# jingsenzhu/i2-sdf

Measured on AMD Instinct MI355X. Metric: ray-samples/sec (fwd+bwd), higher is better.
Workload: dtype f32 (bf16x3 split MFMA: fp32 operands as 3 bf16 terms, fp32 accumulate; the 256x256 weight-gradient GEMM blocks and the sampler's depth-choosing sdf-only passes: 2 bf16 terms per operand, 3 products, fp32 accumulate; the saved SDF tensors abar / G(hbar) / G(a) -- operands of those GEMMs and of the s

## Files before the change

i2sdf_amd/csrc/pack.hip:

```cpp
#include "plan.h"

using namespace i2sdf;

int i2sdf_hip_check(hipError_t e, const char* what);

namespace {

struct RowTab {
  int32_t n;
  int32_t rows[3 * I2SDF_MAX_LAYERS], cols[3 * I2SDF_MAX_LAYERS], scale_off[3 * I2SDF_MAX_LAYERS];
  int64_t off_v[3 * I2SDF_MAX_LAYERS], off_g[3 * I2SDF_MAX_LAYERS];
};

__global__ __launch_bounds__(256) void rowscale_kernel(RowTab tab, const float* __restrict__ params, float* __restrict__ scale,
                                                        int n_rows) {
  const int row = blockIdx.x * 4 + (threadIdx.x >> 6);
  const int lane = threadIdx.x & 63;
  if (row >= n_rows) return;
  int e = 0;
  while (e + 1 < tab.n && row >= tab.scale_off[e + 1]) ++e;
  const int r = row - tab.scale_off[e];
  const int cols = tab.cols[e];
  const float* v = params + tab.off_v[e] + (int64_t)r * cols;
  float s = 0.f;
  for (int c = lane; c < cols; c += 64) { float x = v[c]; s = fmaf(x, x, s); }
#pragma unroll
  for (int o = 32; o > 0; o >>= 1) s += __shfl_xor(s, o);
  if (lane == 0) scale[row] = params[tab.off_g[e] + r] / sqrtf(s);
}

__device__ __forceinline__ int map_col(const ColMap& cm, int kp) {
  if (kp < cm.split) return kp < cm.valid0 ? cm.base0 + kp : -1;
  const int j = kp - cm.split;
  return j < cm.valid1 ? cm.base1 + j : -1;
}

__global__ __launch_bounds__(256) void pack_kernel(const Seg* __restrict__ segs, int n_segs, const float* __restrict__ params,
                                                    const float* __restrict__ scale, float* __restrict__ chunks,
                                                    int64_t total_chunks) {
  const int64_t gid = (int64_t)blockIdx.x * 256 + threadIdx.x;
  const int64_t chunk = gid >> 6;
  const int lane = (int)(gid & 63);
  if (chunk >= total_chunks) return;
  int lo = 0, hi_ = n_segs - 1;
  while (lo < hi_) {
    const int mid = (lo + hi_ + 1) >> 1;
    if (segs[mid].chunk0 <= chunk) lo = mid; else hi_ = mid - 1;
  }
  const Seg s = segs[lo];
  const int c = (int)(chunk - s.chunk0);
  const int i32 = lane & 31, hi = lane >> 5;
  f32x4 out = {0.f, 0.f, 0.f, 0.f};
  if (c < s.used) {
    if (s.type == SEG_BIAS) {
      const int nt = c / 4, q = c % 4;
#pragma unroll
      for (int t = 0; t < 4; ++t) {
        const int r = 32 * nt + 8 * q + 4 * hi + t;
        out[t] = (r < s.nrows) ? params[s.off_bias + s.row_off + r] : 0.f;
      }
    } else if (s.type == SEG_WFWD) {
      const int nt = c / s.KC, kc = c % s.KC;
      const int r = 32 * nt + i32;
      if (r < s.nrows) {
        const int row = s.row_off + r;
        const float sc = scale[s.scale_off + row] * s.mult;
        const float* v = params + s.off_v + (int64_t)row * s.cols;
#pragma unroll
        for (int t = 0; t < 4; ++t) {
          const int col = map_col(s.cm, 8 * kc + 4 * hi + t);
          out[t] = col >= 0 ? v[col] * sc : 0.f;
        }
      }
    } else if (s.type == SEG_WFWD3) {
      const int G = s.NT / 2, w = c >> 1, e = c & 1;
      const int kc = w / (3 * G), g = (w / 3) % G, sp = w % 3;
      const int r = 32 * (2 * g + e) + i32;
      unsigned q[4] = {0u, 0u, 0u, 0u};
      if (r < s.nrows) {
        const int row = s.row_off + r;
        const float sc = scale[s.scale_off + row] * s.mult;
        const float* v = params + s.off_v + (int64_t)row * s.cols;
#pragma unroll
        for (int i = 0; i < 4; ++i) {
          float x[2];
#pragma unroll
          for (int h2 = 0; h2 < 2; ++h2) {
            const int j = 2 * i + h2;
            const int col = map_col(s.cm, 16 * kc + (j & 3) + 8 * (j >> 2) + 4 * hi);
            x[h2] = col >= 0 ? v[col] * sc : 0.f;
          }
          unsigned p0, p1, p2;
          split3_pair(x[0], x[1], p0, p1, p2);
          q[i] = sp == 0 ? p0 : (sp == 1 ? p1 : p2);
        }
      }
// ... 37 lines not shown
      const int arow = 16 * (2 * g + e) + i16;
      const bool fwd = s.type != SEG_WBWD3H;
      const int acol = fwd ? -1 : map_col(s.cm, arow);
      unsigned q[4] = {0u, 0u, 0u, 0u};
      if (fwd ? (arow < s.nrows) : (acol >= 0)) {
#pragma unroll
        for (int i = 0; i < 4; ++i) {
          float x[2];
#pragma unroll
          for (int h2 = 0; h2 < 2; ++h2) {
            const int j = 2 * i + h2;
            const int k = 32 * kc + 16 * (j >> 2) + 4 * kg + (j & 3);
            x[h2] = 0.f;
            if (fwd) {
              const int row = s.row_off + arow, col = map_col(s.cm, k);
              if (col >= 0) x[h2] = params[s.off_v + (int64_t)row * s.cols + col] * (scale[s.scale_off + row] * s.mult);
            } else if (k < s.nrows) {
              const int row = s.row_off + k;
              x[h2] = params[s.off_v + (int64_t)row * s.cols + acol] * scale[s.scale_off + row] * s.mult;
            }
          }
          unsigned p0, p1, p2;
          split3_pair(x[0], x[1], p0, p1, p2);
          q[i] = sp == 0 ? p0 : (sp == 1 ? p1 : p2);
        }
      }
      out = __builtin_bit_cast(f32x4, u32x4{q[0], q[1], q[2], q[3]});
    } else if (s.type == SEG_ROWVEC_H) {
      const int rr = c / s.KC, nt = c % s.KC, kg = lane >> 4;
      const int row = s.row_off + rr;
      const float sc = scale[s.scale_off + row] * s.mult;
#pragma unroll
      for (int t = 0; t < 4; ++t) {
        const int col = map_col(s.cm, 16 * nt + 4 * kg + t);
        out[t] = col >= 0 ? params[s.off_v + (int64_t)row * s.cols + col] * sc : 0.f;
      }
    } else if (s.type == SEG_WBWD) {
      const int kt = c / s.KC, nc = c % s.KC;
      const int col = map_col(s.cm, 32 * kt + i32);
      if (col >= 0) {
#pragma unroll
        for (int t = 0; t < 4; ++t) {
          const int r = 8 * nc + 4 * hi + t;
          if (r < s.nrows) {
            const int row = s.row_off + r;
            out[t] = params[s.off_v + (int64_t)row * s.cols + col] * scale[s.scale_off + row] * s.mult;
          }
        }
      }
    } else if (s.type == SEG_ROWVEC) {
      const int rr = c / s.KC, kc = c % s.KC;
      const int row = s.row_off + rr;
      const float sc = scale[s.scale_off + row] * s.mult;
#pragma unroll
      for (int t = 0; t < 4; ++t) {
        const int col = map_col(s.cm, 8 * kc + 4 * hi + t);
        out[t] = col >= 0 ? params[s.off_v + (int64_t)row * s.cols + col] * sc : 0.f;
      }
    } else if (s.type == SEG_SCALAR) {
#pragma unroll
      for (int t = 0; t < 4; ++t) out[t] = (t < s.nrows) ? params[s.off_bias + s.row_off + t] : 0.f;
    }
  }
  reinterpret_cast<f32x4*>(chunks)[chunk * 64 + lane] = out;
}

void fill_tab(RowTab& tab, const NetPlan& np) {
  for (int l = 0; l < np.d.n_lin; ++l) {
    const int e = tab.n++;
    tab.rows[e] = np.d.out_dim[l]; tab.cols[e] = np.d.in_dim[l]; tab.scale_off[e] = np.scale_off[l];
    tab.off_v[e] = np.d.off_v[l]; tab.off_g[e] = np.d.off_g[l];
  }
}

}

extern "C" int i2sdf_pack_weights(const i2sdf_plan* p, const float* params, float* packed, void* stream) {
  if (!p || !params || !packed) return I2SDF_EINVAL;
  if (!p->d_segs) return I2SDF_EHIP;
  hipStream_t st = (hipStream_t)stream;
  RowTab tab{};
  fill_tab(tab, p->sdf); fill_tab(tab, p->rgb);
  if (p->light.d.n_lin) fill_tab(tab, p->light);
  rowscale_kernel<<<cdiv(p->n_scale, 4), 256, 0, st>>>(tab, params, packed, p->n_scale);
  const int64_t threads = p->total_chunks * 64;
  pack_kernel<<<(unsigned)((threads + 255) / 256), 256, 0, st>>>(p->d_segs, p->n_segs, params, packed, packed + p->scale_floats,
                                                                 p->total_chunks);
  return i2sdf_hip_check(hipGetLastError(), "pack_weights launch");
}
```

i2sdf_amd/csrc/plan.cpp:

```cpp
#include <hip/hip_runtime.h>
#include <string.h>
#include <initializer_list>
#include <string>
#include "plan.h"
#include <stdlib.h>

using namespace i2sdf;

static thread_local std::string g_hip_err;

int i2sdf_hip_check(hipError_t e, const char* what) {
  if (e == hipSuccess) return I2SDF_OK;
  g_hip_err = std::string(what) + ": " + hipGetErrorString(e);
  return I2SDF_EHIP;
}

extern "C" int i2sdf_version(void) { return I2SDF_VERSION; }
extern "C" const char* i2sdf_last_hip_error(void) { return g_hip_err.c_str(); }
extern "C" const char* i2sdf_strerror(int code) {
  switch (code) {
    case I2SDF_OK: return "ok";
    case I2SDF_EINVAL: return "invalid argument or unsupported network shape";
    case I2SDF_EHIP: return "HIP runtime error";
    case I2SDF_ESPHERE: return "ray misses the scene bounding sphere";
// ... 479 lines not shown
  }
  if (option == I2SDF_OPT_WGRAD_BF16X2) {
    p->wgrad_bf16x2 = value ? 1 : 0;
    return I2SDF_OK;
  }
  if (option == I2SDF_OPT_BLOCKED_SAVES) {
    p->blocked_saves = value ? 1 : 0;
    return I2SDF_OK;
  }
  if (option == I2SDF_OPT_SAVES24) {
    if (value && (p->H != 256 || p->F != 256 || span_chunks(p->sdf, SPAN_REV3_CHAIN) == 0)) return I2SDF_EINVAL;
    if (p->chain_active) return I2SDF_EINVAL;
    p->saves24 = value ? 1 : 0;
    return I2SDF_OK;
  }
  if (option == I2SDF_OPT_TAIL_OVERLAP) {
    p->tail_overlap = value ? 1 : 0;
    return I2SDF_OK;
  }
  return I2SDF_EINVAL;
}

extern "C" int i2sdf_plan_set_exchange(i2sdf_plan* p, const i2sdf_exchange* ex, int32_t flags) {
  if (!p || (flags & ~I2SDF_DP_GLOBAL_SAMPLER) || (ex && !ex->allreduce)) return I2SDF_EINVAL;
  p->exchange = ex ? *ex : i2sdf_exchange{nullptr, nullptr};
  p->dp_flags = ex ? flags : 0;
  return I2SDF_OK;
}

extern "C" int64_t i2sdf_plan_pack_floats(const i2sdf_plan* p) {
// ... 4 lines not shown
```

i2sdf_amd/csrc/plan.h:

```cpp
#pragma once
#include <stdint.h>
#include <vector>
#include "../../include/i2sdf.h"
#include "x3h.h"

namespace i2sdf {

enum SegType : int32_t { SEG_ZERO = 0, SEG_BIAS = 1, SEG_WFWD = 2, SEG_WBWD = 3, SEG_ROWVEC = 4, SEG_SCALAR = 5,
                         SEG_WFWD3 = 6 ,
                         SEG_WBWD3 = 7 ,
                         SEG_BIAS_H = 8, SEG_WFWD3H = 9, SEG_WBWD3H = 10, SEG_ROWVEC_H = 11,
                         SEG_WFWD2H = 12  };

struct ColMap { int32_t split, base0, valid0, base1, valid1; };

struct Seg {
  int64_t chunk0;
  int32_t nchunks;
  int32_t type;
  int64_t off_v, off_bias;
  int32_t scale_off;
  int32_t rows, cols;
  int32_t row_off;
  int32_t nrows;
// ... 51 lines not shown
  int64_t wgrad_floats = 0;
  int32_t H = 0, F = 0;
  int32_t n_cu = 256;
  int32_t rgb_bf16x3 = 0;
  int32_t sdf_bwd_bf16x3 = 0;
  int32_t train_fwd_bf16x3 = 0;
  int32_t wgrad_bf16x3 = 0;
  int32_t sdf_fwd_bf16x3 = 0;
  int32_t sampler_bf16x2 = 0;
  i2sdf_exchange exchange{nullptr, nullptr};
  int32_t dp_flags = 0;
  int32_t wgrad_bf16x2 = 0;
  int32_t blocked_saves = 0;
  int32_t saves24 = 0;
  int32_t tail_overlap = 0;
  mutable hipStream_t side = nullptr;
  mutable hipEvent_t ev_fork = nullptr, ev_join = nullptr;
  int32_t parts = 0;
  mutable hipStream_t part_st[I2SDF_MAX_PARTS - 1] = {nullptr, nullptr, nullptr};
  mutable hipEvent_t part_ev[I2SDF_MAX_PARTS] = {nullptr, nullptr, nullptr, nullptr};
  mutable int32_t chain_active = 0;
  mutable int64_t chain_M = 0;
};

namespace i2sdf {
struct Span { const float* w = nullptr; int n_stages = 0; };
inline int64_t span_chunks(const NetPlan& np, SpanId id) { return np.mark[id.to] - np.mark[id.from]; }
inline Span span(const i2sdf_plan* p, const float* packed, const NetPlan& np, SpanId id) {
  const int64_t n = span_chunks(np, id);
  if (n <= 0 || n % id.stage_chunks) return Span{};
// ... 63 lines not shown
```

i2sdf_amd/csrc/sampler.hip:

```cpp
#include "plan.h"

using namespace i2sdf;

int i2sdf_hip_check(hipError_t e, const char* what);

namespace {

constexpr int NMAX = 640;
constexpr int NNEW = 128;
constexpr int EMAX = NMAX / 64;

enum { ST_DONE = 0, ST_ITERS = 1, ST_FLAG0 = 2 , ST_CNT0 = 16 , ST_WORDS = 32 };

#ifndef SAMPLER_DPP
#define SAMPLER_DPP 1
#endif
template <int CTRL, int ROW_MASK>
__device__ __forceinline__ float dpp_mov(float old, float v) {
  return __builtin_bit_cast(float, __builtin_amdgcn_update_dpp(__builtin_bit_cast(int, old), __builtin_bit_cast(int, v), CTRL, ROW_MASK, 0xf, false));
}
constexpr int DPP_ROW_SHR1 = 0x111, DPP_ROW_SHR2 = 0x112, DPP_ROW_SHR4 = 0x114, DPP_ROW_SHR8 = 0x118, DPP_ROW_BCAST15 = 0x142, DPP_ROW_BCAST31 = 0x143;
__device__ __forceinline__ float wscan_incl(float v, int lane) {
#if SAMPLER_DPP
  (void)lane;
// ... 410 lines not shown
          const float x = buf[wv][i], y = buf[wv][l];
          const bool up = (i & k) == 0;
          if ((x > y) == up) { buf[wv][i] = y; buf[wv][l] = x; }
        }
      }
      __syncthreads();
    }
  }
  if (active) {
    for (int k = lane; k < total; k += 64) z_out[ray * ldz + k] = buf[wv][k];
    if (lane == 0 && z_eik) {
      int id = eik_idx ? eik_idx[ray] : 0;
      id = id < 0 ? 0 : (id > total - 1 ? total - 1 : id);
      z_eik[ray] = buf[wv][id];
    }
  }
}

template <int E>
__global__ __launch_bounds__(256) void error_bound_kernel(int64_t B, int n, const float* __restrict__ z, const float* __restrict__ sdf,
                                                           const float* __restrict__ beta, int64_t ldbeta, const float* __restrict__ d_star_in,
                                                           float* __restrict__ d_star_out, float* __restrict__ bound) {
  const int lane = threadIdx.x & 63;
  const int64_t ray = (int64_t)blockIdx.x * 4 + (threadIdx.x >> 6);
  if (ray >= B) return;
  Row<E> r;
  load_row<E>(r, z + ray * n, sdf + ray * n, n, lane);
  row_intervals<E>(r, lane);
#pragma unroll
  for (int e = 0; e < E; ++e) {
// ... 107 lines not shown
    int xrc = I2SDF_OK;
    switch (E) {
      case 1: xrc = launch_iter<1>(a, st, gcomm); break;
      case 2: xrc = launch_iter<2>(a, st, gcomm); break;
      case 3: xrc = launch_iter<3>(a, st, gcomm); break;
      case 4: xrc = launch_iter<4>(a, st, gcomm); break;
      case 5: xrc = launch_iter<5>(a, st, gcomm); break;
      case 6: xrc = launch_iter<6>(a, st, gcomm); break;
      case 7: xrc = launch_iter<7>(a, st, gcomm); break;
      case 8: xrc = launch_iter<8>(a, st, gcomm); break;
      case 9: xrc = launch_iter<9>(a, st, gcomm); break;
      default: xrc = launch_iter<10>(a, st, gcomm); break;
    }
    if (xrc) return xrc;
  }
  sampler_final_kernel<<<grid, 256, 0, st>>>(B, state, sc->N_samples_eval, zA, zB, samples, sc->N_samples, sc->N_samples_extra,
                                             training ? (const int*)extra_idx : nullptr, (const int*)extra_tab, near, far, (const int*)eik_idx, z_out, ldz,
                                             z_eik, iters_out);
  return i2sdf_hip_check(hipGetLastError(), "sample_rays launch");
}
```

i2sdf_amd/engine.py:

```python
from __future__ import annotations

import ctypes as C
from typing import Optional

import os

import torch

from . import lib as L
from .config import NetConfig
from .params import ParamLayout


class RenderEngine:
    def __init__(self, cfg: NetConfig, device="cuda"):
        self.cfg = cfg
        self.layout = ParamLayout(cfg)
        self.device = torch.device(device)
        self._lib = L.load()
        self._desc = self.layout.net_desc()
        plan = C.c_void_p()
        L.check(self._lib.i2sdf_plan_create(C.byref(self._desc), C.byref(plan)), "i2sdf_plan_create")
        self._plan = plan
        self.pack_floats = int(self._lib.i2sdf_plan_pack_floats(plan))
        self.wgrad_floats = int(self._lib.i2sdf_plan_wgrad_floats(plan))
        self.packed = torch.zeros(self.pack_floats, dtype=torch.float32, device=self.device)
        self._pack_stream, self._pack_event, self._pack_readers = None, None, {}
        self.F = cfg.feature_size
        wide = cfg.sdf.hidden == 256 and cfg.feature_size == 256
        self.set_sdf_forward_bf16x3(bool(cfg.bf16x3 and cfg.sdf.hidden % 64 == 0))
        self.set_wgrad_bf16x3(bool(cfg.bf16x3))
        self.set_train_forward_bf16x3(bool(cfg.bf16x3 and wide))
        self.set_sdf_backward_bf16x3(bool(cfg.bf16x3 and wide))
        self.set_rgb_bf16x3(bool(cfg.bf16x3 and cfg.rgb.hidden == 256 and cfg.feature_size == 256 and cfg.rgb.n_lin >= 3))
        self.wgrad_bf16x2 = False
        x2 = os.environ.get("I2SDF_WGRAD_BF16X2", "")
        self.set_wgrad_bf16x2(bool(cfg.bf16x3 and ((x2 != "0") if x2 != "" else cfg.wgrad_bf16x2)))
        self.sampler_bf16x2 = False
        sx2 = os.environ.get("I2SDF_SAMPLER_BF16X2", "")
        if wide:
            self.set_sampler_bf16x2(bool(self.sdf_forward_bf16x3 and ((sx2 != "0") if sx2 != "" else getattr(cfg, "sampler_bf16x2", False))))
        self.set_blocked_saves(bool(cfg.bf16x3 and os.environ.get("I2SDF_BLOCKED_SAVES", "1") != "0"))
        self.saves24 = False
        s24 = os.environ.get("I2SDF_SAVES24", "")
        if wide:
            self.set_saves24(bool(cfg.bf16x3 and ((s24 != "0") if s24 != "" else getattr(cfg, "saves24", True))))
        self.set_tail_overlap(os.environ.get("I2SDF_TAIL_OVERLAP", "1") != "0")
        self.parts = 0
        n_parts = int(os.environ.get("I2SDF_PARTS", "2"))
        self._parts_wanted = n_parts if (cfg.bf16x3 and n_parts >= 2) else 0
        self._sync_parts()
        sc = cfg.sampler
        self._scfg = L.SamplerCfg(near=sc.near, eps=sc.eps, add_tiny=sc.add_tiny, N_samples=sc.N_samples, N_samples_eval=sc.N_samples_eval,
                                  N_samples_extra=sc.N_samples_extra, beta_iters=sc.beta_iters, max_total_iters=sc.max_total_iters)
        dev = self.device
        self.t_lin = torch.linspace(0.0, 1.0, steps=sc.N_samples_eval, device=dev)
        self.u_more = torch.linspace(0.0, 1.0, steps=sc.N_samples_eval, device=dev)
        self.u_final = torch.linspace(0.0, 1.0, steps=sc.N_samples, device=dev)
        if sc.N_samples_extra > 0:
            self.extra_tab = torch.stack([torch.linspace(0, sc.N_samples_eval * (it + 1) - 1, sc.N_samples_extra).long()
                                          for it in range(sc.max_total_iters)]).to(torch.int32).to(dev).contiguous()
# ... 9 lines not shown
            def __init__(self, fn, name):
                self.fn, self.name = fn, name

            def __call__(self, *a):
                e0, e1 = torch.cuda.Event(enable_timing=True), torch.cuda.Event(enable_timing=True)
                e0.record()
                rc = self.fn(*a)
                e1.record()
                eng._timing.append((self.name, e0, e1))
                return rc

        self._timed_lib = type("TimedLib", (), {})()
        for name in L.SIGNATURES:
            fn = getattr(self._lib, name)
            if name in ("i2sdf_sdf_forward", "i2sdf_sdf_forward_grad", "i2sdf_rgb_forward", "i2sdf_rgb_backward", "i2sdf_sdf_backward",
                        "i2sdf_weight_grads", "i2sdf_sample_rays", "i2sdf_composite_forward", "i2sdf_composite_backward", "i2sdf_pack_weights",
                        "i2sdf_ray_setup", "i2sdf_light_forward", "i2sdf_light_backward"):
                fn = _Timed(fn, name)
            setattr(self._timed_lib, name, fn)
        self._real_lib, self._lib = self._lib, self._timed_lib

    def stop_timing(self):
        self._lib = self._real_lib
        out = {}
        for name, e0, e1 in self._timing:
            tot, cnt = out.get(name, (0.0, 0))
            out[name] = (tot + e0.elapsed_time(e1), cnt + 1)
        self._timing = []
        return out

    def __del__(self):
# ... 7 lines not shown
    def pack(self, flat_params: torch.Tensor):
        assert flat_params.is_cuda and flat_params.dtype == torch.float32 and flat_params.numel() == self.layout.n_params
        if os.environ.get("I2SDF_PACK_ASYNC", "1") == "0":
            L.check(self._lib.i2sdf_pack_weights(self._plan, L.ptr(flat_params), L.ptr(self.packed), L.stream_ptr()), "i2sdf_pack_weights")
            return
        dev = flat_params.device
        side = self._pack_stream
        if side is None:
            side = self._pack_stream = torch.cuda.Stream(device=dev)
        cur = torch.cuda.current_stream(dev)
        side.wait_stream(cur)
        for st in getattr(self, "_pack_readers", {}):
            if st != cur:
                side.wait_stream(st)
        with torch.cuda.stream(side):
            L.check(self._lib.i2sdf_pack_weights(self._plan, L.ptr(flat_params), L.ptr(self.packed), L.stream_ptr()), "i2sdf_pack_weights")
            self._pack_event = side.record_event()
        flat_params.record_stream(side)
        self._pack_readers = {}

    def _pk(self):
        ev = self._pack_event
        if ev is not None:
            cur = torch.cuda.current_stream(self.packed.device)
            readers = self.__dict__.setdefault("_pack_readers", {})
            if cur not in readers:
                cur.wait_event(ev)
                readers[cur] = True
        return L.ptr(self.packed)

    def set_sdf_forward_bf16x3(self, on: bool):
        L.check(self._lib.i2sdf_plan_set_option(self._plan, L.OPT_SDF_FWD_BF16X3, int(bool(on))), "i2sdf_plan_set_option")
        self.sdf_forward_bf16x3 = bool(on)

    def set_train_forward_bf16x3(self, on: bool):
        L.check(self._lib.i2sdf_plan_set_option(self._plan, L.OPT_TRAIN_FWD_BF16X3, int(bool(on))), "i2sdf_plan_set_option")
        self.train_forward_bf16x3 = bool(on)
        if hasattr(self, "_parts_wanted"):
            self._sync_parts()

    def set_sdf_backward_bf16x3(self, on: bool):
        L.check(self._lib.i2sdf_plan_set_option(self._plan, L.OPT_SDF_BWD_BF16X3, int(bool(on))), "i2sdf_plan_set_option")
        self.sdf_backward_bf16x3 = bool(on)
        if hasattr(self, "_parts_wanted"):
# ... 286 lines not shown
        return d

    def sample_rays(self, flat_params, cam, dirs, training=False, strat_u=None, cdf_u=None, extra_idx=None, eik_idx=None, force_iters=0):
        B, dev = cam.shape[0], cam.device
        ws = torch.empty(int(self._lib.i2sdf_sampler_workspace_floats(B)), dtype=torch.float32, device=dev)
        z_out = torch.empty(B, self.n_z, dtype=torch.float32, device=dev)
        z_eik = torch.empty(B, 1, dtype=torch.float32, device=dev)
        iters = torch.empty(1, dtype=torch.int32, device=dev) if B > 0 else torch.zeros(1, dtype=torch.int32, device=dev)
        i32 = lambda t: None if t is None else t.to(torch.int32).contiguous()
        if training:
            u_final, ldu = cdf_u.contiguous(), cdf_u.shape[1]
        else:
            u_final, ldu = self.u_final, 0
        ex, ek = i32(extra_idx), i32(eik_idx)
        su = None if strat_u is None else strat_u.contiguous()
        L.check(self._lib.i2sdf_sample_rays(self._plan, self._pk(), L.ptr(flat_params), C.byref(self._scfg), L.ptr(cam.contiguous()),
                                             L.ptr(dirs.contiguous()), B, 1 if training else 0, L.ptr(self.t_lin), L.ptr(self.u_more),
                                             L.ptr(u_final), ldu, L.ptr(self.extra_tab), L.ptr(su), L.ptr(ex), L.ptr(ek), force_iters,
                                             L.ptr(ws), L.ptr(z_out), self.n_z, L.ptr(z_eik), L.ptr(iters), L.stream_ptr()),
                 "i2sdf_sample_rays")
        self._last_sampler_ws = ws
        return z_out, z_eik, iters

    def error_bound(self, z, sdf, beta, d_star=None, want_d_star=False):
        z, sdf = z.detach().float().contiguous(), sdf.detach().float().reshape(z.shape).contiguous()
        B, n = z.shape
        beta = beta.detach().float().reshape(-1).contiguous().to(z.device)
        if beta.numel() not in (1, B):
            raise ValueError("beta must be a scalar or one value per ray")
        bound = torch.empty(B, dtype=torch.float32, device=z.device)
        ds_out = torch.empty(B, n - 1, dtype=torch.float32, device=z.device) if want_d_star else None
        ds_in = None if d_star is None else d_star.detach().float().contiguous()
        L.check(self._lib.i2sdf_error_bound(L.ptr(z), L.ptr(sdf), B, n, L.ptr(beta), 0 if beta.numel() == 1 else 1, L.ptr(ds_in),
                                            L.ptr(ds_out), L.ptr(bound), L.stream_ptr()), "i2sdf_error_bound")
        return (bound, ds_out) if want_d_star else bound
# ... 68 lines not shown
```

i2sdf_amd/lib.py:

```python
from __future__ import annotations

import ctypes as C
import os

MAX_LAYERS = 12
_HERE = os.path.dirname(os.path.abspath(__file__))
LIB_PATH = os.environ.get("I2SDF_LIB_PATH") or os.path.join(_HERE, "lib", "libi2sdf_hip.so")


class MlpDesc(C.Structure):
    _fields_ = [("n_lin", C.c_int32), ("hidden", C.c_int32), ("d_in", C.c_int32), ("in0", C.c_int32), ("d_out", C.c_int32),
                ("multires", C.c_int32), ("skip_layer", C.c_int32), ("reserved", C.c_int32),
                ("out_dim", C.c_int32 * MAX_LAYERS), ("in_dim", C.c_int32 * MAX_LAYERS),
                ("off_bias", C.c_int64 * MAX_LAYERS), ("off_g", C.c_int64 * MAX_LAYERS), ("off_v", C.c_int64 * MAX_LAYERS)]


class NetDesc(C.Structure):
    _fields_ = [("sdf", MlpDesc), ("rgb", MlpDesc), ("light", MlpDesc), ("off_beta", C.c_int64), ("n_params", C.c_int64),
                ("beta_min", C.c_float), ("scene_bounding_sphere", C.c_float)]


class TrainBuffers(C.Structure):
    _fields_ = [("M_sdf", C.c_int64), ("M_main", C.c_int64), ("Mp", C.c_int64)] + [(n, C.c_void_p) for n in (
        "pe", "hs", "abars", "gus", "gpbar", "gas", "ga_last4", "ones4", "fbar", "pev", "feat", "rs", "gar", "ga_last_rgb",
# ... 33 lines not shown
    _fields_ = [(n, C.c_void_p) for n in ("image_idx", "uv", "cam_loc", "dirs", "dnorm", "rgb", "depth", "normal", "mask", "light_mask",
                                          "depth_mask", "normal_mask", "n_bad")]


OPT_SDF_FWD_BF16X3 = 1
OPT_WGRAD_BF16X3 = 2
OPT_TRAIN_FWD_BF16X3 = 4
OPT_SDF_BWD_BF16X3 = 8
OPT_RGB_BF16X3 = 16
OPT_TAIL_OVERLAP = 32
OPT_BLOCKED_SAVES = 128
OPT_WGRAD_BF16X2 = 256
OPT_PARTS = 512
OPT_SAMPLER_BF16X2 = 1024
OPT_SAVES24 = 2048
MAX_PARTS = 4
GRID_ORDER_MESHGRID, GRID_ORDER_VOLUME = 0, 1
RASTER_SMALL_MAX = 64
TSDF_MAX_CELLS = 1 << 24
IMAGE_STATS = 8
SSIM_TILE_X, SSIM_TILE_Y = 32, 16


class I2SDFError(RuntimeError):
    pass


_lib = None

_P, _I64, _I32, _F, _D = C.c_void_p, C.c_int64, C.c_int32, C.c_float, C.c_double
SIGNATURES = {
    "i2sdf_version": (C.c_int, []),
    "i2sdf_strerror": (C.c_char_p, [C.c_int]),
    "i2sdf_last_hip_error": (C.c_char_p, []),
    "i2sdf_plan_create": (C.c_int, [C.POINTER(NetDesc), C.POINTER(_P)]),
    "i2sdf_plan_destroy": (None, [_P]),
    "i2sdf_plan_set_option": (C.c_int, [_P, _I32, _I32]),
    "i2sdf_chain_begin": (C.c_int, [_P, _I64, _P]),
    "i2sdf_chain_fence": (C.c_int, [_P, _P]),
    "i2sdf_chain_end": (C.c_int, [_P, _P]),
    "i2sdf_blocked_points": (_I64, [_P, _I32, _I64, _I64, _I32]),
    "i2sdf_plan_pack_floats": (_I64, [_P]),
    "i2sdf_plan_wgrad_floats": (_I64, [_P]),
    "i2sdf_pack_weights": (C.c_int, [_P, _P, _P, _P]),
    "i2sdf_sdf_forward": (C.c_int, [_P, _P, _P, _I64, _P, _P, _I64, _P]),
    "i2sdf_sdf_forward_grad": (C.c_int, [_P] * 6 + [_I64, _I32, _I64, _I64, _I64] + [_P] * 7),
    "i2sdf_rgb_forward": (C.c_int, [_P, _P, _P, _I32, _P, _I64, _I64, _P, _P, _P, _P]),
    "i2sdf_rgb_backward": (C.c_int, [_P] * 5 + [_I64, _I64] + [_P] * 4),
    "i2sdf_sdf_backward": (C.c_int, [_P] * 6 + [_I64, _I32, _I64, _I64, _I64] + [_P] * 4 + [_I64] + [_P] * 7),
    "i2sdf_wgrad_chunk_points": (_I64, []),
    "i2sdf_weight_grads": (C.c_int, [_P, C.POINTER(TrainBuffers), _P, _P, _I64, _P, _P]),
    "i2sdf_comm_available": (_I32, []),
    "i2sdf_comm_unique_id": (C.c_int, [_P, _I64]),
    "i2sdf_comm_init_rank": (C.c_int, [_P, _I32, _I32, C.POINTER(_P)]),
    "i2sdf_comm_destroy": (None, [_P]),
    "i2sdf_comm_size": (_I32, [_P]),
    "i2sdf_comm_rank": (_I32, [_P]),
    "i2sdf_last_comm_error": (C.c_char_p, []),
    "i2sdf_allreduce_grads": (C.c_int, [_P, _I64, _P, _P]),
# ... 112 lines not shown
```

include/i2sdf.h:

```cpp
#ifndef I2SDF_H
#define I2SDF_H

#include <stddef.h>
#include <stdint.h>

#ifdef __cplusplus
extern "C" {
#endif

#define I2SDF_VERSION 100
#define I2SDF_MAX_LAYERS 12
#define I2SDF_MAX_PARTS 4

#define I2SDF_OK 0
#define I2SDF_EINVAL (-1)
#define I2SDF_EHIP (-2)
#define I2SDF_ESPHERE (-3)
#define I2SDF_EWORKSPACE (-4)
#define I2SDF_ECOMM (-5)

typedef struct i2sdf_mlp_desc {
  int32_t n_lin;
  int32_t hidden;
  int32_t d_in;
// ... 26 lines not shown
const char* i2sdf_last_hip_error(void);

int i2sdf_plan_create(const i2sdf_net_desc* desc, i2sdf_plan** out);
void i2sdf_plan_destroy(i2sdf_plan* plan);
#define I2SDF_OPT_SDF_FWD_BF16X3 1
#define I2SDF_OPT_WGRAD_BF16X3 2
#define I2SDF_OPT_TRAIN_FWD_BF16X3 4
#define I2SDF_OPT_SDF_BWD_BF16X3 8
#define I2SDF_OPT_RGB_BF16X3 16
#define I2SDF_OPT_TAIL_OVERLAP 32
#define I2SDF_OPT_BLOCKED_SAVES 128
#define I2SDF_OPT_WGRAD_BF16X2 256
#define I2SDF_OPT_PARTS 512
#define I2SDF_OPT_SAMPLER_BF16X2 1024
#define I2SDF_OPT_SAVES24 2048
int64_t i2sdf_blocked_points(const i2sdf_plan* plan, int32_t which, int64_t M, int64_t Mp, int32_t has_feat);
int i2sdf_plan_set_option(i2sdf_plan* plan, int32_t option, int32_t value);
int i2sdf_chain_begin(const i2sdf_plan* plan, int64_t M, void* stream);
int i2sdf_chain_fence(const i2sdf_plan* plan, void* stream);
int i2sdf_chain_end(const i2sdf_plan* plan, void* stream);
int64_t i2sdf_plan_pack_floats(const i2sdf_plan* plan);
int64_t i2sdf_plan_wgrad_floats(const i2sdf_plan* plan);

int i2sdf_pack_weights(const i2sdf_plan* plan, const float* params, float* packed, void* stream);

int i2sdf_sdf_forward(const i2sdf_plan* plan, const float* packed, const float* points, int64_t M,
                      float* sdf_out, float* feat_out, int64_t ld_feat, void* stream);


int i2sdf_sdf_forward_grad(const i2sdf_plan* plan, const float* packed, const float* points, const float* cam,
                           const float* dirs, const float* z, int64_t ldz, int32_t n_per_ray, int64_t n_ray_pts, int64_t M,
                           int64_t Mp, float* sdf, float* feat, float* grad, float* hs, float* abars, float* pe_save,
                           void* stream);

int i2sdf_rgb_forward(const i2sdf_plan* plan, const float* packed, const float* dirs, int32_t n_per_ray, const float* feat,
                      int64_t M, int64_t Mp, float* rgb, float* rs, float* pev_save, void* stream);

int i2sdf_rgb_backward(const i2sdf_plan* plan, const float* packed, const float* rgb, const float* rgb_bar, const float* rs,
                       int64_t M, int64_t Mp, float* gar, float* ga_last, float* fbar, void* stream);
// ... 273 lines not shown
```

Measured before the change: 20.89 million.

## Split weight packing into sampler head and tail; add rank-based final sample sort

Measured after the change: 20.89 million (median of 3 runs). Within noise of the previous version (+0.0%).

```diff
diff --git a/i2sdf_amd/csrc/pack.hip b/i2sdf_amd/csrc/pack.hip
--- a/i2sdf_amd/csrc/pack.hip
+++ b/i2sdf_amd/csrc/pack.hip
@@ -12,21 +12,52 @@
   int64_t off_v[3 * I2SDF_MAX_LAYERS], off_g[3 * I2SDF_MAX_LAYERS];
 };
 
+template <int NB>
+__device__ __forceinline__ void wave_row_scales(const float* __restrict__ v0, const float* __restrict__ g0, int cols, int n, int lane,
+                                                float (&sc)[NB]) {
+  float s[NB];
+#pragma unroll
+  for (int u = 0; u < NB; ++u) {
+    const float* v = v0 + (int64_t)(u < n ? u : n - 1) * cols;
+    s[u] = 0.f;
+#pragma unroll
+    for (int q = 0; q < 5; ++q) {
+      const int c = lane + 64 * q;
+      const float x = c < cols ? v[c] : 0.f;
+      s[u] = fmaf(x, x, s[u]);
+    }
+    for (int c = lane + 320; c < cols; c += 64) { const float x = v[c]; s[u] = fmaf(x, x, s[u]); }
+  }
+#pragma unroll
+  for (int o = 32; o > 0; o >>= 1) {
+#pragma unroll
+    for (int u = 0; u < NB; ++u) s[u] += __shfl_xor(s[u], o);
+  }
+#pragma unroll
+  for (int u = 0; u < NB; ++u) sc[u] = g0[u < n ? u : n - 1] / sqrtf(s[u]);
+}
+
+__device__ __forceinline__ int tab_entry(const RowTab& tab, int row) {
+  int e = 0;
+  while (e + 1 < tab.n && row >= tab.scale_off[e + 1]) ++e;
+  return e;
+}
+
+__device__ __forceinline__ float wave_row_scale(const RowTab& tab, const float* __restrict__ params, int row, int lane) {
+  const int e = tab_entry(tab, row);
+  const int r = row - tab.scale_off[e];
+  float sc[1];
+  wave_row_scales<1>(params + tab.off_v[e] + (int64_t)r * tab.cols[e], params + tab.off_g[e] + r, tab.cols[e], 1, lane, sc);
+  return sc[0];
+}
+
 __global__ __launch_bounds__(256) void rowscale_kernel(RowTab tab, const float* __restrict__ params, float* __restrict__ scale,
                                                         int n_rows) {
   const int row = blockIdx.x * 4 + (threadIdx.x >> 6);
   const int lane = threadIdx.x & 63;
   if (row >= n_rows) return;
-  int e = 0;
-  while (e + 1 < tab.n && row >= tab.scale_off[e + 1]) ++e;
-  const int r = row - tab.scale_off[e];
-  const int cols = tab.cols[e];
-  const float* v = params + tab.off_v[e] + (int64_t)r * cols;
-  float s = 0.f;
-  for (int c = lane; c < cols; c += 64) { float x = v[c]; s = fmaf(x, x, s); }
-#pragma unroll
-  for (int o = 32; o > 0; o >>= 1) s += __shfl_xor(s, o);
-  if (lane == 0) scale[row] = params[tab.off_g[e] + r] / sqrtf(s);
+  const float sc = wave_row_scale(tab, params, row, lane);
+  if (lane == 0) scale[row] = sc;
 }
 
 __device__ __forceinline__ int map_col(const ColMap& cm, int kp) {
@@ -35,20 +66,31 @@
   return j < cm.valid1 ? cm.base1 + j : -1;
 }
 
-__global__ __launch_bounds__(256) void pack_kernel(const Seg* __restrict__ segs, int n_segs, const float* __restrict__ params,
-                                                    const float* __restrict__ scale, float* __restrict__ chunks,
-                                                    int64_t total_chunks) {
-  const int64_t gid = (int64_t)blockIdx.x * 256 + threadIdx.x;
-  const int64_t chunk = gid >> 6;
-  const int lane = (int)(gid & 63);
-  if (chunk >= total_chunks) return;
+__device__ __forceinline__ int find_seg(const Seg* __restrict__ segs, int n_segs, int64_t chunk) {
   int lo = 0, hi_ = n_segs - 1;
   while (lo < hi_) {
     const int mid = (lo + hi_ + 1) >> 1;
     if (segs[mid].chunk0 <= chunk) lo = mid; else hi_ = mid - 1;
   }
-  const Seg s = segs[lo];
-  const int c = (int)(chunk - s.chunk0);
+  return lo;
+}
+
+__device__ __forceinline__ int lane_scale_row(const Seg& s, int c, int lane) {
+  if (c >= s.used) return -1;
+  int r = -1;
+  if (s.type == SEG_WFWD) r = 32 * (c / s.KC) + (lane & 31);
+  else if (s.type == SEG_WFWD3) r = 32 * (2 * (((c >> 1) / 3) % (s.NT / 2)) + (c & 1)) + (lane & 31);
+  else if (s.type == SEG_WFWD3H || s.type == SEG_WFWD2H) {
+    const int PL = s.type == SEG_WFWD2H ? 2 : 3;
+    r = 16 * (2 * (((c >> 1) / PL) % (s.NT / 2)) + (c & 1)) + (lane & 15);
+  } else if (s.type == SEG_ROWVEC || s.type == SEG_ROWVEC_H) return s.scale_off + s.row_off + c / s.KC;
+  else return -1;
+  return r < s.nrows ? s.scale_off + s.row_off + r : -1;
+}
+
+template <bool OWN>
+__device__ __forceinline__ f32x4 pack_chunk_lane(const Seg& s, int c, int lane, const float* __restrict__ params, const float* __restrict__ scale,
+                                                 float own_scale) {
   const int i32 = lane & 31, hi = lane >> 5;
   f32x4 out = {0.f, 0.f, 0.f, 0.f};
   if (c < s.used) {
@@ -64,7 +106,7 @@
       const int r = 32 * nt + i32;
       if (r < s.nrows) {
         const int row = s.row_off + r;
-        const float sc = scale[s.scale_off + row] * s.mult;
+        const float sc = (OWN ? own_scale : scale[s.scale_off + row]) * s.mult;
         const float* v = params + s.off_v + (int64_t)row * s.cols;
 #pragma unroll
         for (int t = 0; t < 4; ++t) {
@@ -79,7 +121,7 @@
       unsigned q[4] = {0u, 0u, 0u, 0u};
       if (r < s.nrows) {
         const int row = s.row_off + r;
-        const float sc = scale[s.scale_off + row] * s.mult;
+        const float sc = (OWN ? own_scale : scale[s.scale_off + row]) * s.mult;
         const float* v = params + s.off_v + (int64_t)row * s.cols;
 #pragma unroll
         for (int i = 0; i < 4; ++i) {
@@ -147,7 +189,7 @@
             x[h2] = 0.f;
             if (fwd) {
               const int row = s.row_off + arow, col = map_col(s.cm, k);
-              if (col >= 0) x[h2] = params[s.off_v + (int64_t)row * s.cols + col] * (scale[s.scale_off + row] * s.mult);
+              if (col >= 0) x[h2] = params[s.off_v + (int64_t)row * s.cols + col] * ((OWN ? own_scale : scale[s.scale_off + row]) * s.mult);
             } else if (k < s.nrows) {
               const int row = s.row_off + k;
               x[h2] = params[s.off_v + (int64_t)row * s.cols + acol] * scale[s.scale_off + row] * s.mult;
@@ -162,7 +204,7 @@
     } else if (s.type == SEG_ROWVEC_H) {
       const int rr = c / s.KC, nt = c % s.KC, kg = lane >> 4;
       const int row = s.row_off + rr;
-      const float sc = scale[s.scale_off + row] * s.mult;
+      const float sc = (OWN ? own_scale : scale[s.scale_off + row]) * s.mult;
 #pragma unroll
       for (int t = 0; t < 4; ++t) {
         const int col = map_col(s.cm, 16 * nt + 4 * kg + t);
@@ -184,7 +226,7 @@
     } else if (s.type == SEG_ROWVEC) {
       const int rr = c / s.KC, kc = c % s.KC;
       const int row = s.row_off + rr;
-      const float sc = scale[s.scale_off + row] * s.mult;
+      const float sc = (OWN ? own_scale : scale[s.scale_off + row]) * s.mult;
 #pragma unroll
       for (int t = 0; t < 4; ++t) {
         const int col = map_col(s.cm, 8 * kc + 4 * hi + t);
@@ -195,7 +237,56 @@
       for (int t = 0; t < 4; ++t) out[t] = (t < s.nrows) ? params[s.off_bias + s.row_off + t] : 0.f;
     }
   }
-  reinterpret_cast<f32x4*>(chunks)[chunk * 64 + lane] = out;
+  return out;
+}
+
+__global__ __launch_bounds__(256) void pack_kernel(const Seg* __restrict__ segs, int n_segs, const float* __restrict__ params,
+                                                    const float* __restrict__ scale, float* __restrict__ chunks,
+                                                    int64_t total_chunks, int64_t skip_lo, int64_t skip_hi) {
+  const int64_t gid = (int64_t)blockIdx.x * 256 + threadIdx.x;
+  int64_t chunk = gid >> 6;
+  const int lane = (int)(gid & 63);
+  if (chunk >= skip_lo) chunk += skip_hi - skip_lo;
+  if (chunk >= total_chunks) return;
+  const Seg s = segs[find_seg(segs, n_segs, chunk)];
+  reinterpret_cast<f32x4*>(chunks)[chunk * 64 + lane] = pack_chunk_lane<false>(s, (int)(chunk - s.chunk0), lane, params, scale, 0.f);
+}
+
+__global__ __launch_bounds__(256) void pack_head_kernel(RowTab tab, int n_rows, int scale_blocks, const Seg* __restrict__ segs, int n_segs,
+                                                         const float* __restrict__ params, float* __restrict__ scale, float* __restrict__ chunks,
+                                                         int64_t g_lo, int64_t g_hi) {
+  const int lane = threadIdx.x & 63, wv = __builtin_amdgcn_readfirstlane(threadIdx.x >> 6);
+  if ((int)blockIdx.x < scale_blocks) {
+    const int row = blockIdx.x * 4 + wv;
+    if (row >= n_rows) return;
+    const float sc = wave_row_scale(tab, params, row, lane);
+    if (lane == 0) scale[row] = sc;
+    return;
+  }
+  const int64_t chunk = g_lo + (int64_t)(blockIdx.x - scale_blocks) * 4 + wv;
+  if (chunk >= g_hi) return;
+  const Seg s = segs[find_seg(segs, n_segs, chunk)];
+  const int c = (int)(chunk - s.chunk0);
+  const int need = lane_scale_row(s, c, lane);
+  const bool rowvec = s.type == SEG_ROWVEC || s.type == SEG_ROWVEC_H;
+  const int T = (s.type == SEG_WFWD3H || s.type == SEG_WFWD2H) ? 16 : 32;
+  const int first = __builtin_amdgcn_readfirstlane(need);
+  const int count = first < 0 ? 0 : (rowvec ? 1 : __popcll(__ballot(need >= 0) & ((1ull << T) - 1)));
+  float own = 0.f;
+  if (count > 0) {
+    const int e = tab_entry(tab, first);
+    const int r0 = first - tab.scale_off[e], cols = tab.cols[e];
+    const float* v0 = params + tab.off_v[e] + (int64_t)r0 * cols;
+    const float* g0 = params + tab.off_g[e] + r0;
+    constexpr int NB = 8;
+    for (int b = 0; b < count; b += NB) {
+      float sc[NB];
+      wave_row_scales<NB>(v0 + (int64_t)b * cols, g0 + b, cols, count - b, lane, sc);
+#pragma unroll
+      for (int u = 0; u < NB; ++u) own = (need == first + b + u) ? sc[u] : own;
+    }
+  }
+  reinterpret_cast<f32x4*>(chunks)[chunk * 64 + lane] = pack_chunk_lane<true>(s, c, lane, params, scale, own);
 }
 
 void fill_tab(RowTab& tab, const NetPlan& np) {
@@ -206,18 +297,51 @@
   }
 }
 
+void head_range(const i2sdf_plan* p, int64_t* lo, int64_t* hi) {
+  SpanId id = SPAN_FWD_SDF;
+  if (p->sdf_fwd_bf16x3 && p->H == 256 && span_chunks(p->sdf, SPAN_FWD3H) > 0)
+    id = (p->sampler_bf16x2 && span_chunks(p->sdf, SPAN_FWD2H) > 0) ? SPAN_FWD2H : SPAN_FWD3H_SDF;
+  else if (p->sdf_fwd_bf16x3 && p->H == 64 && span_chunks(p->sdf, SPAN_FWD3) > 0)
+    id = SPAN_FWD3;
+  *lo = p->sdf.mark[id.from]; *hi = p->sdf.mark[id.to];
+}
+
+int pack_launch(const i2sdf_plan* p, const float* params, float* packed, int part, hipStream_t st) {
+  RowTab tab{};
+  fill_tab(tab, p->sdf); fill_tab(tab, p->rgb);
+  if (p->light.d.n_lin) fill_tab(tab, p->light);
+  float* chunks = packed + p->scale_floats;
+  if (!p->pack_split) {
+    if (part == 1) return I2SDF_OK;
+    rowscale_kernel<<<cdiv(p->n_scale, 4), 256, 0, st>>>(tab, params, packed, p->n_scale);
+    const int64_t threads = p->total_chunks * 64;
+    pack_kernel<<<(unsigned)((threads + 255) / 256), 256, 0, st>>>(p->d_segs, p->n_segs, params, packed, chunks, p->total_chunks, p->total_chunks, p->total_chunks);
+    return i2sdf_hip_check(hipGetLastError(), "pack_weights launch");
+  }
+  int64_t g_lo = 0, g_hi = 0;
+  head_range(p, &g_lo, &g_hi);
+  if (part != 1) {
+    const int scale_blocks = cdiv(p->n_scale, 4);
+    pack_head_kernel<<<(unsigned)(scale_blocks + (g_hi - g_lo + 3) / 4), 256, 0, st>>>(tab, p->n_scale, scale_blocks, p->d_segs, p->n_segs, params, packed,
+                                                                                      chunks, g_lo, g_hi);
+  }
+  if (part != 0) {
+    const int64_t threads = (p->total_chunks - (g_hi - g_lo)) * 64;
+    pack_kernel<<<(unsigned)((threads + 255) / 256), 256, 0, st>>>(p->d_segs, p->n_segs, params, packed, chunks, p->total_chunks, g_lo, g_hi);
+  }
+  return i2sdf_hip_check(hipGetLastError(), "pack_weights launch");
+}
+
 }
 
 extern "C" int i2sdf_pack_weights(const i2sdf_plan* p, const float* params, float* packed, void* stream) {
   if (!p || !params || !packed) return I2SDF_EINVAL;
   if (!p->d_segs) return I2SDF_EHIP;
-  hipStream_t st = (hipStream_t)stream;
-  RowTab tab{};
-  fill_tab(tab, p->sdf); fill_tab(tab, p->rgb);
-  if (p->light.d.n_lin) fill_tab(tab, p->light);
-  rowscale_kernel<<<cdiv(p->n_scale, 4), 256, 0, st>>>(tab, params, packed, p->n_scale);
-  const int64_t threads = p->total_chunks * 64;
-  pack_kernel<<<(unsigned)((threads + 255) / 256), 256, 0, st>>>(p->d_segs, p->n_segs, params, packed, packed + p->scale_floats,
-                                                                 p->total_chunks);
-  return i2sdf_hip_check(hipGetLastError(), "pack_weights launch");
-}
+  return pack_launch(p, params, packed, -1, (hipStream_t)stream);
+}
+
+extern "C" int i2sdf_pack_weights_part(const i2sdf_plan* p, const float* params, float* packed, int32_t part, void* stream) {
+  if (!p || !params || !packed || (part != 0 && part != 1)) return I2SDF_EINVAL;
+  if (!p->d_segs) return I2SDF_EHIP;
+  return pack_launch(p, params, packed, part, (hipStream_t)stream);
+}
diff --git a/i2sdf_amd/csrc/plan.cpp b/i2sdf_amd/csrc/plan.cpp
--- a/i2sdf_amd/csrc/plan.cpp
+++ b/i2sdf_amd/csrc/plan.cpp
@@ -517,6 +517,14 @@
     p->saves24 = value ? 1 : 0;
     return I2SDF_OK;
   }
+  if (option == I2SDF_OPT_PACK_SPLIT) {
+    p->pack_split = value ? 1 : 0;
+    return I2SDF_OK;
+  }
+  if (option == I2SDF_OPT_FINAL_RANKSORT) {
+    p->final_ranksort = value ? 1 : 0;
+    return I2SDF_OK;
+  }
   if (option == I2SDF_OPT_TAIL_OVERLAP) {
     p->tail_overlap = value ? 1 : 0;
     return I2SDF_OK;
diff --git a/i2sdf_amd/csrc/plan.h b/i2sdf_amd/csrc/plan.h
--- a/i2sdf_amd/csrc/plan.h
+++ b/i2sdf_amd/csrc/plan.h
@@ -89,6 +89,8 @@
   int32_t blocked_saves = 0;
   int32_t saves24 = 0;
   int32_t tail_overlap = 0;
+  int32_t pack_split = 1;
+  int32_t final_ranksort = 1;
   mutable hipStream_t side = nullptr;
   mutable hipEvent_t ev_fork = nullptr, ev_join = nullptr;
   int32_t parts = 0;
diff --git a/i2sdf_amd/csrc/sampler.hip b/i2sdf_amd/csrc/sampler.hip
--- a/i2sdf_amd/csrc/sampler.hip
+++ b/i2sdf_amd/csrc/sampler.hip
@@ -448,6 +448,66 @@
       id = id < 0 ? 0 : (id > total - 1 ? total - 1 : id);
       z_eik[ray] = buf[wv][id];
     }
+  }
+}
+
+__global__ __launch_bounds__(256) void sampler_final_rank_kernel(int64_t B, const int* __restrict__ state, int N_eval, const float* z_a,
+                                                                  const float* z_b, const float* __restrict__ samples, int N_final, int N_extra,
+                                                                  const int* __restrict__ extra_idx, const int* __restrict__ extra_tab,
+                                                                  float near, float far, const int* __restrict__ eik_idx, float* __restrict__ z_out,
+                                                                  int64_t ldz, float* __restrict__ z_eik, int* __restrict__ iters_out) {
+  const int lane = threadIdx.x & 63, wv = threadIdx.x >> 6;
+  const int64_t ray = (int64_t)blockIdx.x * 4 + wv;
+  const int iters = state[ST_ITERS];
+  if (iters_out != nullptr && blockIdx.x == 0 && threadIdx.x == 0) iters_out[0] = iters;
+  if (ray >= B) return;
+  const int n_row = N_eval * iters;
+  const float* zr = ((iters & 1) ? z_a : z_b) + ray * NMAX;
+  const int total = N_final + 2 + N_extra;
+  float key[2];
+#pragma unroll
+  for (int h = 0; h < 2; ++h) {
+    const int k = lane + 64 * h;
+    float v = 3.0e38f;
+    if (k < N_final) v = samples[ray * NNEW + k];
+    else if (k == N_final) v = near;
+    else if (k == N_final + 1) v = far;
+    else if (k < total) {
+      const int e = k - N_final - 2;
+      int id;
+      if (extra_idx) id = extra_idx[(iters - 1) * N_extra + e];
+      else id = extra_tab[(iters - 1) * N_extra + e];
+      id = id < 0 ? 0 : (id > n_row - 1 ? n_row - 1 : id);
+      v = zr[id];
+    }
+    key[h] = v;
+  }
+  int rank0 = 0, rank1 = 0;
+#pragma unroll
+  for (int j = 0; j < 64; ++j) {
+    const float a = __builtin_bit_cast(float, __builtin_amdgcn_readlane(__builtin_bit_cast(int, key[0]), j));
+    rank0 += (a < key[0] || (a == key[0] && j < lane)) ? 1 : 0;
+    rank1 += (a <= key[1]) ? 1 : 0;
+  }
+  if (total > 64) {
+#pragma unroll
+    for (int j = 0; j < 64; ++j) {
+      const float b = __builtin_bit_cast(float, __builtin_amdgcn_readlane(__builtin_bit_cast(int, key[1]), j));
+      rank0 += (b < key[0]) ? 1 : 0;
+      rank1 += (b < key[1] || (b == key[1] && j < lane)) ? 1 : 0;
+    }
+  } else {
+    rank1 = 64 + lane;
+  }
+  int id = eik_idx ? eik_idx[ray] : 0;
+  id = id < 0 ? 0 : (id > total - 1 ? total - 1 : id);
+  if (rank0 < total) {
+    z_out[ray * ldz + rank0] = key[0];
+    if (z_eik && rank0 == id) z_eik[ray] = key[0];
+  }
+  if (rank1 < total) {
+    z_out[ray * ldz + rank1] = key[1];
+    if (z_eik && rank1 == id) z_eik[ray] = key[1];
   }
 }
 
@@ -585,8 +645,13 @@
     }
     if (xrc) return xrc;
   }
-  sampler_final_kernel<<<grid, 256, 0, st>>>(B, state, sc->N_samples_eval, zA, zB, samples, sc->N_samples, sc->N_samples_extra,
-                                             training ? (const int*)extra_idx : nullptr, (const int*)extra_tab, near, far, (const int*)eik_idx, z_out, ldz,
-                                             z_eik, iters_out);
+  if (p->final_ranksort && sc->N_samples + 2 + sc->N_samples_extra <= 128)
+    sampler_final_rank_kernel<<<grid, 256, 0, st>>>(B, state, sc->N_samples_eval, zA, zB, samples, sc->N_samples, sc->N_samples_extra,
+                                                    training ? (const int*)extra_idx : nullptr, (const int*)extra_tab, near, far, (const int*)eik_idx,
+                                                    z_out, ldz, z_eik, iters_out);
+  else
+    sampler_final_kernel<<<grid, 256, 0, st>>>(B, state, sc->N_samples_eval, zA, zB, samples, sc->N_samples, sc->N_samples_extra,
+                                               training ? (const int*)extra_idx : nullptr, (const int*)extra_tab, near, far, (const int*)eik_idx, z_out, ldz,
+                                               z_eik, iters_out);
   return i2sdf_hip_check(hipGetLastError(), "sample_rays launch");
 }
diff --git a/i2sdf_amd/engine.py b/i2sdf_amd/engine.py
--- a/i2sdf_amd/engine.py
+++ b/i2sdf_amd/engine.py
@@ -26,6 +26,7 @@
         self.wgrad_floats = int(self._lib.i2sdf_plan_wgrad_floats(plan))
         self.packed = torch.zeros(self.pack_floats, dtype=torch.float32, device=self.device)
         self._pack_stream, self._pack_event, self._pack_readers = None, None, {}
+        self._pack_head_event = None
         self.F = cfg.feature_size
         wide = cfg.sdf.hidden == 256 and cfg.feature_size == 256
         self.set_sdf_forward_bf16x3(bool(cfg.bf16x3 and cfg.sdf.hidden % 64 == 0))
@@ -45,6 +46,8 @@
         s24 = os.environ.get("I2SDF_SAVES24", "")
         if wide:
             self.set_saves24(bool(cfg.bf16x3 and ((s24 != "0") if s24 != "" else getattr(cfg, "saves24", True))))
+        self.set_pack_split(os.environ.get("I2SDF_PACK_SPLIT", "1") != "0")
+        self.set_final_ranksort(os.environ.get("I2SDF_FINAL_RANKSORT", "1") != "0")
         self.set_tail_overlap(os.environ.get("I2SDF_TAIL_OVERLAP", "1") != "0")
         self.parts = 0
         n_parts = int(os.environ.get("I2SDF_PARTS", "2"))
@@ -84,7 +87,7 @@
         for name in L.SIGNATURES:
             fn = getattr(self._lib, name)
             if name in ("i2sdf_sdf_forward", "i2sdf_sdf_forward_grad", "i2sdf_rgb_forward", "i2sdf_rgb_backward", "i2sdf_sdf_backward",
-                        "i2sdf_weight_grads", "i2sdf_sample_rays", "i2sdf_composite_forward", "i2sdf_composite_backward", "i2sdf_pack_weights",
+                        "i2sdf_weight_grads", "i2sdf_sample_rays", "i2sdf_composite_forward", "i2sdf_composite_backward", "i2sdf_pack_weights", "i2sdf_pack_weights_part",
                         "i2sdf_ray_setup", "i2sdf_light_forward", "i2sdf_light_backward"):
                 fn = _Timed(fn, name)
             setattr(self._timed_lib, name, fn)
@@ -122,20 +125,38 @@
             if st != cur:
                 side.wait_stream(st)
         with torch.cuda.stream(side):
-            L.check(self._lib.i2sdf_pack_weights(self._plan, L.ptr(flat_params), L.ptr(self.packed), L.stream_ptr()), "i2sdf_pack_weights")
-            self._pack_event = side.record_event()
+            if self.pack_split:
+                L.check(self._lib.i2sdf_pack_weights_part(self._plan, L.ptr(flat_params), L.ptr(self.packed), 0, L.stream_ptr()), "i2sdf_pack_weights_part")
+                self._pack_head_event = side.record_event()
+                L.check(self._lib.i2sdf_pack_weights_part(self._plan, L.ptr(flat_params), L.ptr(self.packed), 1, L.stream_ptr()), "i2sdf_pack_weights_part")
+                self._pack_event = side.record_event()
+            else:
+                L.check(self._lib.i2sdf_pack_weights(self._plan, L.ptr(flat_params), L.ptr(self.packed), L.stream_ptr()), "i2sdf_pack_weights")
+                self._pack_head_event = self._pack_event = side.record_event()
         flat_params.record_stream(side)
         self._pack_readers = {}
-
-    def _pk(self):
+        self._pack_head_key = (self.sdf_forward_bf16x3, self.sampler_bf16x2)
+
+    def _pk(self, head_only: bool = False):
         ev = self._pack_event
         if ev is not None:
             cur = torch.cuda.current_stream(self.packed.device)
             readers = self.__dict__.setdefault("_pack_readers", {})
-            if cur not in readers:
-                cur.wait_event(ev)
-                readers[cur] = True
+            if head_only and getattr(self, "_pack_head_key", None) != (self.sdf_forward_bf16x3, self.sampler_bf16x2):
+                head_only = False
+            want = 1 if head_only else 2
+            if readers.get(cur, 0) < want:
+                cur.wait_event(self._pack_head_event if head_only else ev)
+                readers[cur] = want
         return L.ptr(self.packed)
+
+    def set_pack_split(self, on: bool):
+        L.check(self._lib.i2sdf_plan_set_option(self._plan, L.OPT_PACK_SPLIT, int(bool(on))), "i2sdf_plan_set_option")
+        self.pack_split = bool(on)
+
+    def set_final_ranksort(self, on: bool):
+        L.check(self._lib.i2sdf_plan_set_option(self._plan, L.OPT_FINAL_RANKSORT, int(bool(on))), "i2sdf_plan_set_option")
+        self.final_ranksort = bool(on)
 
     def set_sdf_forward_bf16x3(self, on: bool):
         L.check(self._lib.i2sdf_plan_set_option(self._plan, L.OPT_SDF_FWD_BF16X3, int(bool(on))), "i2sdf_plan_set_option")
@@ -452,11 +473,12 @@
             u_final, ldu = self.u_final, 0
         ex, ek = i32(extra_idx), i32(eik_idx)
         su = None if strat_u is None else strat_u.contiguous()
-        L.check(self._lib.i2sdf_sample_rays(self._plan, self._pk(), L.ptr(flat_params), C.byref(self._scfg), L.ptr(cam.contiguous()),
+        L.check(self._lib.i2sdf_sample_rays(self._plan, self._pk(head_only=True), L.ptr(flat_params), C.byref(self._scfg), L.ptr(cam.contiguous()),
                                              L.ptr(dirs.contiguous()), B, 1 if training else 0, L.ptr(self.t_lin), L.ptr(self.u_more),
                                              L.ptr(u_final), ldu, L.ptr(self.extra_tab), L.ptr(su), L.ptr(ex), L.ptr(ek), force_iters,
                                              L.ptr(ws), L.ptr(z_out), self.n_z, L.ptr(z_eik), L.ptr(iters), L.stream_ptr()),
                  "i2sdf_sample_rays")
+        self._pk()
         self._last_sampler_ws = ws
         return z_out, z_eik, iters
 
diff --git a/i2sdf_amd/lib.py b/i2sdf_amd/lib.py
--- a/i2sdf_amd/lib.py
+++ b/i2sdf_amd/lib.py
@@ -71,6 +71,8 @@
 OPT_PARTS = 512
 OPT_SAMPLER_BF16X2 = 1024
 OPT_SAVES24 = 2048
+OPT_FINAL_RANKSORT = 8192
+OPT_PACK_SPLIT = 16384
 MAX_PARTS = 4
 GRID_ORDER_MESHGRID, GRID_ORDER_VOLUME = 0, 1
 RASTER_SMALL_MAX = 64
@@ -100,6 +102,7 @@
     "i2sdf_plan_pack_floats": (_I64, [_P]),
     "i2sdf_plan_wgrad_floats": (_I64, [_P]),
     "i2sdf_pack_weights": (C.c_int, [_P, _P, _P, _P]),
+    "i2sdf_pack_weights_part": (C.c_int, [_P, _P, _P, _I32, _P]),
     "i2sdf_sdf_forward": (C.c_int, [_P, _P, _P, _I64, _P, _P, _I64, _P]),
     "i2sdf_sdf_forward_grad": (C.c_int, [_P] * 6 + [_I64, _I32, _I64, _I64, _I64] + [_P] * 7),
     "i2sdf_rgb_forward": (C.c_int, [_P, _P, _P, _I32, _P, _I64, _I64, _P, _P, _P, _P]),
diff --git a/include/i2sdf.h b/include/i2sdf.h
--- a/include/i2sdf.h
+++ b/include/i2sdf.h
@@ -64,6 +64,8 @@
 #define I2SDF_OPT_PARTS 512
 #define I2SDF_OPT_SAMPLER_BF16X2 1024
 #define I2SDF_OPT_SAVES24 2048
+#define I2SDF_OPT_FINAL_RANKSORT 8192
+#define I2SDF_OPT_PACK_SPLIT 16384
 int64_t i2sdf_blocked_points(const i2sdf_plan* plan, int32_t which, int64_t M, int64_t Mp, int32_t has_feat);
 int i2sdf_plan_set_option(i2sdf_plan* plan, int32_t option, int32_t value);
 int i2sdf_chain_begin(const i2sdf_plan* plan, int64_t M, void* stream);
@@ -73,6 +75,7 @@
 int64_t i2sdf_plan_wgrad_floats(const i2sdf_plan* plan);
 
 int i2sdf_pack_weights(const i2sdf_plan* plan, const float* params, float* packed, void* stream);
+int i2sdf_pack_weights_part(const i2sdf_plan* plan, const float* params, float* packed, int32_t part, void* stream);
 
 int i2sdf_sdf_forward(const i2sdf_plan* plan, const float* packed, const float* points, int64_t M,
                       float* sdf_out, float* feat_out, int64_t ld_feat, void* stream);
```
